# rhysnewell/Lorikeet

Measured on AMD Instinct MI355X. Metric: PairHMM cell-updates/s (GCUPS), higher is better.
Workload: dtype f64; 1 GPU; config2 x 1024 regions per GPU: 128 reads x 8 haps, R=150, H=300; regions_per_gpu=1024, seed=1000, env=PHMM_REGION_OWN_QUEUE=0 in this process only

## Files before the change

### lorikeet_amd/csrc/phmm_chain_kernels.hip

```cpp
#include "phmm_device.hpp"

namespace phmm {

namespace {

#ifndef PHMM_CHAIN_L
#define PHMM_CHAIN_L 16
#endif
constexpr int CL = PHMM_CHAIN_L;
#ifndef PHMM_RING
#define PHMM_RING 256
#endif
constexpr int RING = PHMM_RING;
constexpr int RING_SLOTS = RING + 4 + 1;
constexpr int CHAIN_META = CHAIN_MAX_READS + 8;
constexpr uint32_t X_PAD = 0x100u;
constexpr uint32_t X_NONE = 0x102u;
constexpr int LEAD = CL - 1;

__device__ __forceinline__ double from_left_inject(double v, double inject, bool group_head) {
    constexpr int ctrl = CL == 16 ? 0x111 : 0x138;
    int lo = __builtin_amdgcn_update_dpp(__double2loint(inject), __double2loint(v), ctrl, 0xf, 0xf, false);
    int hi = __builtin_amdgcn_update_dpp(__double2hiint(inject), __double2hiint(v), ctrl, 0xf, 0xf, false);
    if constexpr (CL == 32) {
        lo = group_head ? __double2loint(inject) : lo;
        hi = group_head ? __double2hiint(inject) : hi;
    }
    return __hiloint2double(hi, lo);
}

template <int K>
__device__ __forceinline__ void chain_fallback(const ForwardParams &p, const ChainItem &it, RowConst *ring, int lane,
                                               int grp, int l, const HapCols<K> &hc, int H, bool hv, int a, int Nh) {
    const uint32_t reg = it.region;
    for (uint32_t r = it.read_begin; r < it.read_end; ++r) {
        const uint32_t ro = p.read_off[r];
        const int R = (int)(p.read_off[r + 1] - ro);
        bool z = false;
        for (int row = lane; row < R; row += WAVE) z |= row_blocks_prescale(p, ro + row);
        const bool scaled = __ballot(z) == 0ull;
        const bool staged = R + 1 <= RING;
        lds_wave_sync();
        if (staged) {
            if (lane == 0) ring[0] = neutral_row();
            for (int row = lane; row < R; row += WAVE) ring[row + 1] = make_row(p, ro, row, R, scaled);
        }
        lds_wave_sync();
        const double scale0 = (scaled && R > 0) ? 1.0 - p.eps[p.gcp[ro]] : 1.0;
        const double fin = (scaled && R > 0) ? 1.0 - p.eps[p.base_q[ro + R - 1]] : 1.0;
        const double c0 = p.initial_condition / (double)H * scale0;
        const bool group_head = (CL == 32) && (lane == 32);
        double s = staged ? sweep_general<CL, K>(LdsView{ring}, R, l, group_head, hc, H, c0, scaled, fin)
                          : sweep_general<CL, K>(GlobalRowView{p, ro, R, scaled}, R, l, group_head, hc, H, c0, scaled, fin);
#pragma unroll
        for (int off = CL / 2; off > 0; off >>= 1) s += __shfl_xor(s, off, WAVE);
        if (l == 0 && hv) {
            const double v = log10(s) - p.initial_condition_log10;
            p.out[p.out_off[reg] + (uint64_t)(r - p.region_read_off[reg]) * (uint64_t)Nh + a] = v;
            if (const uint32_t sb = status_bits(v)) atomicOr(p.status, sb);
        }
    }
    (void)grp;
}

template <int K>
__device__ __forceinline__ void chain_fallback_streams(const ForwardParams &p, uint32_t reg, uint32_t r_begin, int n_mine,
                                                       int n_iter, int lane, int l, const HapCols<K> &hc, int H, bool hv,
                                                       int a, int Nh) {
    const uint64_t group_bits = 0xffffull << (lane & ~15);
    for (int i = 0; i < n_iter; ++i) {
        const bool valid = i < n_mine;
        const uint32_t r = r_begin + (uint32_t)i;
        const uint32_t ro = valid ? p.read_off[r] : 0u;
        const int R = valid ? (int)(p.read_off[r + 1] - ro) : 0;
        bool z = false;
        for (int row = l; row < R; row += 16) z |= row_blocks_prescale(p, ro + row);
        const bool scaled = (__ballot(z) & group_bits) == 0ull;
        const double scale0 = (scaled && R > 0) ? 1.0 - p.eps[p.gcp[ro]] : 1.0;
        const double fin = (scaled && R > 0) ? 1.0 - p.eps[p.base_q[ro + R - 1]] : 1.0;
        const double c0 = p.initial_condition / (double)H * scale0;
        double s = sweep_general<16, K>(GlobalRowView{p, ro, R, scaled}, R, l, false, hc, H, c0, scaled, fin);
#pragma unroll
        for (int off = 8; off > 0; off >>= 1) s += __shfl_xor(s, off, WAVE);
        if (l == 0 && hv && valid) {
            const double v = log10(s) - p.initial_condition_log10;
            p.out[p.out_off[reg] + (uint64_t)(r - p.region_read_off[reg]) * (uint64_t)Nh + a] = v;
            if (const uint32_t sb = status_bits(v)) atomicOr(p.status, sb);
        }
    }
}

}

template <int CLT, int K, int MODE = CHAIN_PLAIN>
__device__ __forceinline__ void chain_body(const ForwardParams &p, const ChainItem it, unsigned char *smem, const ChainItemX *x = nullptr,
                                           double *park = nullptr) {
    static_assert(CLT == CL, "one lanes-per-pair value per compilation unit");
    static_assert(MODE == CHAIN_PLAIN || CL == 16, "prefix sharing: 16 lanes per pair");
    const int col0 = MODE == CHAIN_SUFFIX ? (int)x->mask_or_col0 : 0;
    const uint32_t park_rows = MODE == CHAIN_PLAIN ? 0u : 16u * x->park_rows16;
    const uint32_t park_mask = MODE == CHAIN_PARK ? (uint32_t)x->mask_or_col0 : 0u;
    const int lane = threadIdx.x;
    const int grp = lane / CL, l = lane % CL;
    const bool group_head = (CL == 32) && (lane == 32);
    const uint32_t reg = it.region;
    const int n_chain = (int)(it.read_end - it.read_begin);
    const uint32_t h0 = p.region_hap_off[reg];
    const int Nh = (int)(p.region_hap_off[reg + 1] - h0);
    const int S = (CL == 16) ? (int)it.streams : 1;
    const int GS = (WAVE / CL) / S;
    const int sid = grp / GS;
    const int a = MODE == CHAIN_PLAIN ? (int)it.quad * GS + grp % GS : (int)x->hap[grp & 3];
    const bool hv = a < Nh;
    const int n_sub = (n_chain + S - 1) / S;
    const int TPS = (RING / 4) / S;
    const int NM = RING / S - 1;
    auto n_of = [&](int s) { return max(0, min(n_sub, n_chain - s * n_sub)); };
    const int n_mine = n_of(sid);
    uint32_t ho = 0;
    int H = 0;
    if (hv) {
        ho = p.hap_off[h0 + a];
        H = (int)(p.hap_off[h0 + a + 1] - ho);
    }
    RowConst *ring = reinterpret_cast<RowConst *>(smem);
    uint32_t *roff = reinterpret_cast<uint32_t *>(ring + RING_SLOTS);
    uint32_t *stot = roff + CHAIN_META;

    HapCols<K> hc;
    bool lane_n = false;
#pragma unroll
    for (int w = 0; w < HapCols<K>::W; ++w) hc.y[w] = 0u;
#pragma unroll
    for (int k = 0; k < K; ++k) {
        const int col = col0 + l * K + k;
        uint32_t y = col < H ? (uint32_t)p.hap_bases[ho + col] : X_PAD;
        const bool is_n = (y == 'N');
        lane_n |= is_n;
        hc.set(k, y);
    }

    const uint32_t rb = it.read_begin;
    const uint32_t byte0 = p.read_off[rb];
    const uint32_t bytes = p.read_off[it.read_end] - byte0;
    bool z = false;
    for (uint32_t i = lane; i < bytes; i += WAVE) z |= row_blocks_prescale(p, byte0 + i);
    if ((__ballot(z) | __ballot(lane_n)) != 0ull) {
        if constexpr (MODE == CHAIN_SUFFIX) {
            for (uint32_t r = rb + (uint32_t)l; r < it.read_end && hv; r += CL)
                p.out[p.out_off[reg] + (uint64_t)(r - p.region_read_off[reg]) * (uint64_t)Nh + a] = __longlong_as_double(0x7ff8000000000000ll);
            if (lane == 0) atomicOr(p.status, STATUS_RESCUE);
            return;
        }
        if (S == 1)
            chain_fallback<K>(p, it, ring, lane, grp, l, hc, H, hv, a, Nh);
        else if constexpr (CL == 16)
            chain_fallback_streams<K>(p, reg, rb + (uint32_t)(sid * n_sub), n_mine, n_sub, lane, l, hc, H, hv, a, Nh);
        return;
    }
    {
        const int sj = lane / n_sub, ij = lane % n_sub;
        uint32_t len = lane < n_chain ? p.read_off[rb + lane + 1] - p.read_off[rb + lane] + 2u : 0u;
        uint32_t incl = len;
#pragma unroll
        for (int off = 1; off < WAVE; off <<= 1) {
            const uint32_t v = __shfl_up(incl, off, WAVE);
            if (lane >= off) incl += v;
        }
        const uint32_t before = __shfl(incl, max(sj * n_sub - 1, 0), WAVE);
        const int cb = sj * (n_sub + 1);
        if (lane < 4) stot[lane] = 0u;
        if (lane < n_chain) {
            roff[cb + ij] = p.read_off[rb + lane];
            if (ij + 1 == n_of(sj)) {
                roff[cb + ij + 1] = p.read_off[rb + lane + 1];
                stot[sj] = incl - (sj > 0 ? before : 0u);
            }
        }
        if (lane == 0) ring[RING_SLOTS - 1] = neutral_row();
    }
    lds_wave_sync();
    const int S_max = (int)max(max(stot[0], stot[1]), max(stot[2], stot[3]));
    const double c_unit = ldexp(1.0, 1010);

    uint32_t pb_x = 0, pb_q = 0, pb_qp = 0, pb_i = 0, pb_d = 0, pb_dp = 0, pb_g = 0, pb_gn = 0;
    double pb_bM = 0.0, pb_bD = 0.0;
    int p_Q = 0;
    const bool producer = lane < S * TPS;
    const int ps = producer ? lane / TPS : 0, pj = lane % TPS;
    const int pcb = ps * (n_sub + 1), pn = n_of(ps);
    int p_lo = 0, p_row = pj - LEAD - TPS;
    p_Q = pj - TPS;
    uint32_t p_ro = pn > 0 ? roff[pcb] : 0u;
    int p_R = pn > 0 ? (int)(roff[pcb + 1] - p_ro) : 0;
    auto advance = [&]() {
        p_row += TPS;
        p_Q += TPS;
        while (p_lo < pn && p_row >= p_R + 2) {
            p_row -= p_R + 2;
            ++p_lo;
            if (p_lo < pn) {
                p_ro = roff[pcb + p_lo];
                p_R = (int)(roff[pcb + p_lo + 1] - p_ro);
            }
        }
    };
    auto issue = [&]() {
        advance();
        const int row = p_row, R = p_R;
        const uint32_t ro = p_ro;
        if constexpr (MODE == CHAIN_SUFFIX) {
            if (producer && p_lo < pn && row >= 0 && (uint32_t)p_Q < park_rows) {
                const double *at = park + 2 * ((size_t)x->park_row0 + (size_t)p_Q);
                pb_bM = at[0];
                pb_bD = at[1];
            }
        }
        if (producer && p_lo < pn && row >= 0 && row <= R) {
            pb_qp = row > 0 ? (uint32_t)p.base_q[ro + row - 1] : 0u;
            if (row < R) {
                pb_x = p.read_bases[ro + row];
                pb_q = p.base_q[ro + row];
                pb_i = p.ins_q[ro + row];
                pb_d = p.del_q[ro + row];
                pb_dp = row > 0 ? (uint32_t)p.del_q[ro + row - 1] : 0u;
                pb_g = p.gcp[ro + row];
                pb_gn = row + 1 < R ? (uint32_t)p.gcp[ro + row + 1] : 0u;
            }
        }
    };
    auto finish = [&](int Q0) {
        const int Q = Q0 + pj;
        const int lo = p_lo, row = p_row, R = p_R;
        RowConst n;
        if (lo < pn && row >= 0) {
            if (row < R) {
                n = make_row_bytes(p, pb_x, pb_q, pb_qp, pb_i, pb_d, pb_dp, pb_g, pb_gn, row == 0, row + 1 >= R, true);
            } else if (row == R) {
                n.mm = 1.0 - p.eps[pb_qp]; n.bI = n.mm; n.gI = 1.0; n.dDp = 0.0; n.dd = 1.0; n.pm = 1.0; n.px = 1.0;
                n.x = X_PAD; n.pad0 = (uint32_t)lo; n.pad1 = 0.0;
            } else {
                n.mm = 0.0; n.bI = 0.0; n.gI = 0.0; n.dDp = 0.0; n.dd = 1.0; n.pm = 0.0; n.px = 0.0;
                n.x = X_NONE; n.pad0 = 0;
                n.pad1 = c_unit * (lo + 1 < pn ? 1.0 - p.eps[p.gcp[roff[pcb + lo + 1]]] : 1.0);
            }
            if constexpr (MODE == CHAIN_SUFFIX) {
                n.pm = pb_bM;
                n.pad1 = pb_bD;
            }
        } else {
            n = neutral_row();
        }
        if (producer) {
            const int slot = ps * (NM + 2) + (Q & NM);
            ring[slot] = n;
            if ((Q & NM) == 0) ring[slot + NM + 1] = n;
        }
    };
    issue();
    finish(0);
    issue();
    finish(TPS);
    issue();
    finish(2 * TPS);
    lds_wave_sync();
    issue();

    const double c0 = c_unit * (n_mine > 0 ? 1.0 - p.eps[p.gcp[roff[sid * (n_sub + 1)]]] : 1.0);
    double Mp[K], Ip[K], Dp[K];
#pragma unroll
    for (int k = 0; k < K; ++k) {
        Mp[k] = 0.0;
        Ip[k] = 0.0;
        Dp[k] = c0;
    }
    double aM, aI, aD, bM = 0.0, bI = 0.0, bD = c0;
    const int edge_lane = (H > col0 ? H - 1 - col0 : 0) / K, edge_k = (H > col0 ? H - 1 - col0 : 0) % K;
    const bool last_lane = (l == edge_lane);
    const uint32_t sum_code = last_lane ? X_PAD : 0xffffffffu;
    const double log10_scale = log10(c_unit) + log10((double)H);
    auto emit = [&](const RowConst &c) {
        {
            if (last_lane && c.x == X_PAD && hv) {
                const uint32_t r = rb + (uint32_t)(sid * n_sub) + c.pad0;
                int ek = edge_k;
                asm volatile("" : "+v"(ek));
                double sum = 0.0;
#pragma unroll
                for (int k = 0; k < K; ++k)
                    if (k == ek) sum = (Dp[k] + Mp[k]) + Ip[k];
                const double v = log10(sum) - log10_scale;
                p.out[p.out_off[reg] + (uint64_t)(r - p.region_read_off[reg]) * (uint64_t)Nh + a] = v;
                if (const uint32_t sb = status_bits(v)) atomicOr(p.status, sb);
            }
        }
    };

    int q = LEAD - l;
    const int my_ring = sid * (NM + 2);
    const uint32_t my_rows = (uint32_t)(uintptr_t)(ring + my_ring);
    RowConst cA = lds_row(ring, my_ring + (q & NM)), cB;
    int q1 = q + 1;
    const int T = (S_max + CL - 1 + 1) & ~1;
    bool park_lane = false;
    double2 *park_at = nullptr;
    if constexpr (MODE == CHAIN_PARK) {
        park_lane = grp == 0 && ((park_mask >> l) & 1u) != 0u && hv && (uint32_t)(q + T) <= park_rows;
        const int b = __popc(park_mask & ((1u << l) - 1u));
        park_at = reinterpret_cast<double2 *>(park) + ((size_t)x->park_row0 + (size_t)b * park_rows + (size_t)q);
    }
    const int phase = (int)((blockIdx.x * 2654435761u) >> 26) & (TPS - 2);
    for (int t0 = 0, t1 = min(T, TPS - phase), tick = 0; t0 < T; t0 = t1, t1 = min(T, t1 + TPS), ++tick) {
        if (tick >= 1) {
            finish(TPS * tick + 2 * TPS);
            lds_wave_sync();
            issue();
        }
        for (int t = t0; t < t1; t += 2) {
            uint32_t pair_at;
            asm("v_mad_u32_u24 %0, %1, %2, %3" : "=v"(pair_at) : "v"((uint32_t)(q1 & NM)), "s"((uint32_t)sizeof(RowConst)), "v"(my_rows));
            cB = lds_row_at(pair_at, 0);
            if constexpr (MODE == CHAIN_SUFFIX) {
                aI = from_left_inject(Ip[K - 1], fma(bM, cA.bI, bI * cA.gI), group_head);
                aM = from_left_inject(Mp[K - 1], cA.pm, group_head);
            } else {
                aM = from_left<CL>(Mp[K - 1], group_head);
                aI = from_left<CL>(Ip[K - 1], group_head);
            }
            aD = from_left_inject(Dp[K - 1], cA.pad1, group_head);
            row_update<K, ROW_FAST_EXEC>(Mp, Ip, Dp, bM, bI, bD, aM, aD, cA, hc, 1.0);
            if constexpr (MODE == CHAIN_PARK)
                if (park_lane) park_at[0] = make_double2(Mp[K - 1], Dp[K - 1]);
            if (__ballot(cA.x == sum_code) != 0ull) emit(cA);
            cA = lds_row_at(pair_at, 1);
            if constexpr (MODE == CHAIN_SUFFIX) {
                bI = from_left_inject(Ip[K - 1], fma(aM, cB.bI, aI * cB.gI), group_head);
                bM = from_left_inject(Mp[K - 1], cB.pm, group_head);
            } else {
                bM = from_left<CL>(Mp[K - 1], group_head);
                bI = from_left<CL>(Ip[K - 1], group_head);
            }
            bD = from_left_inject(Dp[K - 1], cB.pad1, group_head);
            row_update<K, ROW_FAST_EXEC>(Mp, Ip, Dp, aM, aI, aD, bM, bD, cB, hc, 1.0);
            if constexpr (MODE == CHAIN_PARK) {
                if (park_lane) park_at[1] = make_double2(Mp[K - 1], Dp[K - 1]);
                park_at += 2;
            }
            if (__ballot(cB.x == sum_code) != 0ull) emit(cB);
            q1 += 2;
        }
    }
}


#define PHMM_CHAIN_K_LIST(X) \
    X(2) X(3) X(4) X(5) X(6) X(7) X(8) X(9) X(10) X(11) X(12) X(13) X(14) X(15) X(16) X(17) X(18) X(19) X(20) X(21) X(22) \
    X(23) X(24) X(25)

template <int CLT, int KLO, int KHI>
__global__ __launch_bounds__(WAVE, 2) void phmm_forward_chain(const ChainParams cp) {
    extern __shared__ __attribute__((aligned(16))) unsigned char smem[];
    const ChainItem it = cp.items[blockIdx.x];
    switch (__builtin_amdgcn_readfirstlane((int)it.k)) {
#define PHMM_CASE(KK)                                                  \
    case KK:                                                           \
        if constexpr (KK >= KLO && KK <= KHI) chain_body<CLT, KK>(cp.f, it, smem); \
        break;
        PHMM_CHAIN_K_LIST(PHMM_CASE)
#undef PHMM_CASE
        default:
            break;
    }
}

template <int CLT, int K>
__global__ __launch_bounds__(WAVE, 2) void phmm_forward_chain_k(const ChainParams cp) {
    extern __shared__ __attribute__((aligned(16))) unsigned char smem[];
    chain_body<CLT, K>(cp.f, cp.items[blockIdx.x], smem);
}

#define PHMM_CHAIN_CAT2(a, b) a##b
#define PHMM_CHAIN_CAT(a, b) PHMM_CHAIN_CAT2(a, b)
#define PHMM_CHAIN_LAUNCH PHMM_CHAIN_CAT(launch_chain_L, PHMM_CHAIN_L)

hipError_t PHMM_CHAIN_LAUNCH(int single_k, const ChainParams &cp, hipStream_t stream) {
    const size_t lds = (size_t)RING_SLOTS * sizeof(RowConst) + (CHAIN_META + 4) * sizeof(uint32_t);
#define PHMM_CASE(KK)                                                                                     \
    if (single_k == KK) {                                                                                 \
        hipLaunchKernelGGL((phmm_forward_chain_k<CL, KK>), dim3(cp.n_items), dim3(WAVE), lds, stream, cp); \
        return hipGetLastError();                                                                         \
    }
    PHMM_CHAIN_K_LIST(PHMM_CASE)
#undef PHMM_CASE
#define PHMM_RANGE(R, LO, HI)                                                                                       \
    if (single_k == -(R + 1)) {                                                                                     \
        hipLaunchKernelGGL((phmm_forward_chain<CL, LO, HI>), dim3(cp.n_items), dim3(WAVE), lds, stream, cp);        \
        return hipGetLastError();                                                                                   \
    }
    PHMM_CHAIN_RANGES(PHMM_RANGE)
#undef PHMM_RANGE
    return hipErrorInvalidValue;
}

#if PHMM_CHAIN_L == 16
hipError_t launch_chain_L32(int single_k, const ChainParams &cp, hipStream_t stream);
hipError_t launch_chain_L64(int single_k, const ChainParams &cp, hipStream_t stream);
int chain_max_k() { return 25; }
hipError_t launch_chain(int L, int single_k, const ChainParams &cp, hipStream_t stream) {
    if (!cp.n_items) return hipSuccess;
    return L == 16 ? launch_chain_L16(single_k, cp, stream) : L == 32 ? launch_chain_L32(single_k, cp, stream)
         : L == 64 ? launch_chain_L64(single_k, cp, stream) : hipErrorInvalidValue;
}
#endif

}
```

### lorikeet_amd/csrc/phmm_device.hpp

```cpp
#pragma once
#include "phmm_internal.hpp"

#include <type_traits>

#ifndef PHMM_SDWA_MIN_K
#define PHMM_SDWA_MIN_K 21
#endif
#ifndef PHMM_CND_MAX_K
#define PHMM_CND_MAX_K 13
#endif
#ifndef PHMM_TWO_WAVE_MAX_K
#define PHMM_TWO_WAVE_MAX_K 25
#endif

namespace phmm {

__device__ __forceinline__ int dpp_row_shr1(int v) {
    return __builtin_amdgcn_update_dpp(0, v, 0x111, 0xf, 0xf, true);
}
__device__ __forceinline__ int dpp_wave_shr1(int v) {
    return __builtin_amdgcn_update_dpp(0, v, 0x138, 0xf, 0xf, true);
}

template <int L>
__device__ __forceinline__ double from_left(double v, bool group_head) {
    int lo = __double2loint(v), hi = __double2hiint(v);
    if constexpr (L == 16) {
        lo = dpp_row_shr1(lo);
        hi = dpp_row_shr1(hi);
    } else {
        lo = dpp_wave_shr1(lo);
        hi = dpp_wave_shr1(hi);
        if constexpr (L == 32) {
            lo = group_head ? 0 : lo;
            hi = group_head ? 0 : hi;
        }
    }
    return __hiloint2double(hi, lo);
}

struct alignas(8) RowConst {
    double mm, bI, gI, dDp, dd, pm, px;
    uint32_t x, pad0;
    double pad1;
};
static_assert(sizeof(RowConst) == 72, "LDS row record");

__device__ __forceinline__ RowConst lds_row(const RowConst *rows, int idx) {
    return *reinterpret_cast<const RowConst *>(reinterpret_cast<const unsigned char *>(rows) +
                                               __mul24(idx, (int)sizeof(RowConst)));
}

__device__ __forceinline__ RowConst lds_row_at(uint32_t at, int skip) {
    RowConst r;
#if defined(__HIP_DEVICE_COMPILE__)
    typedef const __attribute__((address_space(3))) unsigned long long *LdsU64;
    const LdsU64 w = (LdsU64)(uintptr_t)at + skip * (int)(sizeof(RowConst) / 8);
    unsigned long long v[sizeof(RowConst) / 8];
#pragma unroll
    for (int i = 0; i < (int)(sizeof(RowConst) / 8) - 1; ++i) v[i] = w[i];
    v[8] = w[8];
    __builtin_memcpy(&r, v, sizeof r);
#else
    (void)at;
    (void)skip;
    r = RowConst{};
#endif
    return r;
}

struct LdsView {
    const RowConst *rows;
    __device__ __forceinline__ RowConst load(int idx) const { return lds_row(rows, idx); }
};

template <int K, class F>
__device__ __forceinline__ void static_for_down(F &&f) {
    if constexpr (K > 0) {
        f(std::integral_constant<int, K - 1>{});
        static_for_down<K - 1>(f);
    }
}

template <int K>
struct HapCols {
    static constexpr int W = (K + 1) / 2;
    uint32_t y[W];
    __device__ __forceinline__ uint16_t base(int k) const { return (uint16_t)(y[k >> 1] >> (16 * (k & 1))); }
    __device__ __forceinline__ void set(int k, uint32_t yv) { y[k >> 1] |= yv << (16 * (k & 1)); }
};

enum : int { ROW_GENERAL = 0, ROW_FAST_CND = 1, ROW_FAST_EXEC = 2, ROW_FAST_EXEC_PRED = 3 };

template <int K, int MODE>
__device__ __forceinline__ void row_update(double (&Mp)[K], double (&Ip)[K], double (&Dp)[K], const double plM,
                                           const double plI, const double plD, const double lM, const double lD,
                                           const RowConst &c, const HapCols<K> &hc, const double imx,
                                           const uint64_t live = ~0ull) {
    const uint16_t x16 = (uint16_t)c.x;
    if constexpr (MODE == ROW_FAST_EXEC || MODE == ROW_FAST_EXEC_PRED) {
        const uint64_t restore = (MODE == ROW_FAST_EXEC) ? ~0ull : live;
        constexpr bool packed = K > PHMM_SDWA_MIN_K;
        constexpr bool pred = MODE == ROW_FAST_EXEC_PRED;
        uint64_t mask;
        {
            constexpr int k = K - 1;
            const uint32_t y = packed ? hc.y[k >> 1] : (uint32_t)hc.base(k);
            if constexpr (packed && (k & 1))
                asm volatile("v_cmp_ne_u32_sdwa %0, %1, %2 src0_sel:DWORD src1_sel:WORD_1" : "=s"(mask) : "v"(c.x), "v"(y));
            else if constexpr (packed)
                asm volatile("v_cmp_ne_u32_sdwa %0, %1, %2 src0_sel:DWORD src1_sel:WORD_0" : "=s"(mask) : "v"(c.x), "v"(y));
            else
                asm volatile("v_cmp_ne_u32_e64 %0, %1, %2" : "=s"(mask) : "v"(c.x), "v"(y));
        }
        Ip[K - 1] = fma(Mp[K - 1], c.bI, Ip[K - 1] * c.gI);
        static_for_down<K>([&](auto kc) {
            constexpr int k = decltype(kc)::value;
            constexpr int km1 = k > 0 ? k - 1 : 0;
            const uint32_t yn = packed ? hc.y[km1 >> 1] : (uint32_t)hc.base(km1);
            uint64_t next;
#define PHMM_CELL(CMP, RESTORE)                                                                                      \
    asm volatile("v_fma_f64 %[M], %[Dl], %[dDp], %[Il]\n\t"                                                        \
                 "v_fma_f64 %[M], %[Ml], %[mm], %[M]\n\t"                                                          \
                 "s_mov_b64 exec, %[mk]\n\t"                                                                       \
                 "v_mul_f64 %[M], %[px], %[M]\n\t"                                                                 \
                 "s_mov_b64 exec, " RESTORE "\n\t"                                                                 \
                 CMP "\n\t"                                                                                      \
                 "v_mul_f64 %[Il], %[Il], %[gI]\n\t"                                                               \
                 "v_fma_f64 %[Il], %[Ml], %[bI], %[Il]"                                                             \
                 : [M] "=&v"(Mp[k]), [Il] "+v"(Ip[km1]), [mn] "=&s"(next)                                           \
                 : [Dl] "v"(Dp[km1]), [dDp] "v"(c.dDp), [Ml] "v"(Mp[km1]), [mm] "v"(c.mm), [x] "v"(c.x), [y] "v"(yn), \
                   [px] "v"(c.px), [gI] "v"(c.gI), [bI] "v"(c.bI), [live] "s"(restore), [mk] "s"(mask))
            if constexpr (k > 0 && pred && packed && (km1 & 1)) {
                PHMM_CELL("v_cmp_ne_u32_sdwa %[mn], %[x], %[y] src0_sel:DWORD src1_sel:WORD_1", "%[live]");
            } else if constexpr (k > 0 && pred && packed) {
                PHMM_CELL("v_cmp_ne_u32_sdwa %[mn], %[x], %[y] src0_sel:DWORD src1_sel:WORD_0", "%[live]");
            } else if constexpr (k > 0 && pred) {
                PHMM_CELL("v_cmp_ne_u32_e64 %[mn], %[x], %[y]", "%[live]");
            } else if constexpr (k > 0 && packed && (km1 & 1)) {
                PHMM_CELL("v_cmp_ne_u32_sdwa %[mn], %[x], %[y] src0_sel:DWORD src1_sel:WORD_1", "-1");
            } else if constexpr (k > 0 && packed) {
                PHMM_CELL("v_cmp_ne_u32_sdwa %[mn], %[x], %[y] src0_sel:DWORD src1_sel:WORD_0", "-1");
            } else if constexpr (k > 0) {
                PHMM_CELL("v_cmp_ne_u32_e64 %[mn], %[x], %[y]", "-1");
#undef PHMM_CELL
            } else {
                (void)yn;
                double m = fma(plM, c.mm, fma(plD, c.dDp, plI));
                asm volatile("s_mov_b64 exec, %2\n\t"
                             "v_mul_f64 %0, %1, %0\n\t"
                             "s_mov_b64 exec, %3"
                             : "+v"(m)
                             : "v"(c.px), "s"(mask), "s"(restore));
                Mp[0] = m;
                next = 0;
            }
            mask = next;
        });
        double leftM = lM, leftD = lD;
#pragma unroll
        for (int k = 0; k < K; ++k) {
            Dp[k] = fma(leftD, c.dd, leftM);
            leftM = Mp[k];
            leftD = Dp[k];
        }
        return;
    }
    static_for_down<K>([&](auto kc) {
        constexpr int k = decltype(kc)::value;
        Ip[k] = fma(Mp[k], c.bI, Ip[k] * c.gI);
        constexpr int km1 = k > 0 ? k - 1 : 0;
        const double dM = k > 0 ? Mp[km1] : plM;
        const double dI = k > 0 ? Ip[km1] : plI;
        const double dD = k > 0 ? Dp[km1] : plD;
        double t = fma(dD, c.dDp, dI);
        if constexpr (MODE == ROW_GENERAL) t *= imx;
        const double a = fma(dM, c.mm, t);
        const uint16_t yb = hc.base(k);
        const double prior = (x16 == yb || (MODE == ROW_GENERAL && yb == (uint16_t)'N')) ? c.pm : c.px;
        Mp[k] = prior * a;
    });
    double leftM = lM, leftD = lD;
#pragma unroll
    for (int k = 0; k < K; ++k) {
        Dp[k] = fma(leftD, c.dd, leftM);
        leftM = Mp[k];
        leftD = Dp[k];
    }
}


template <int L, int K, int STEADY = ROW_FAST_EXEC>
__device__ __forceinline__ double sweep_fast(const LdsView &lds, const int R, const int l, const bool group_head,
                                             const HapCols<K> &hc, const int H, const double c0, const double fin) {
    double Mp[K], Ip[K], Dp[K];
#pragma unroll
    for (int k = 0; k < K; ++k) {
        Mp[k] = 0.0;
        Ip[k] = 0.0;
        Dp[k] = c0;
    }
    double aM, aI, aD, bM = 0.0, bI = 0.0, bD = c0;
    int row = -l;
    RowConst cA = lds.load(max(row + 1, 0)), cB;
    int t = 0;
    for (; t + 1 < R; t += 2) {
        cB = lds.load(max(row + 2, 0));
        aM = from_left<L>(Mp[K - 1], group_head);
        aI = from_left<L>(Ip[K - 1], group_head);
        aD = from_left<L>(Dp[K - 1], group_head);
        row_update<K, STEADY>(Mp, Ip, Dp, bM, bI, bD, aM, aD, cA, hc, 1.0);
        cA = lds.load(max(row + 3, 0));
        bM = from_left<L>(Mp[K - 1], group_head);
        bI = from_left<L>(Ip[K - 1], group_head);
        bD = from_left<L>(Dp[K - 1], group_head);
        row_update<K, STEADY>(Mp, Ip, Dp, aM, aI, aD, bM, bD, cB, hc, 1.0);
        row += 2;
    }
    RowConst cur = cA;
    double plM = bM, plI = bI, plD = bD;
    if (t < R) {
        const RowConst nxt = lds.load(max(row + 2, 0));
        const double lM = from_left<L>(Mp[K - 1], group_head);
        const double lI = from_left<L>(Ip[K - 1], group_head);
        const double lD = from_left<L>(Dp[K - 1], group_head);
        row_update<K, STEADY>(Mp, Ip, Dp, plM, plI, plD, lM, lD, cur, hc, 1.0);
        plM = lM;
        plI = lI;
        plD = lD;
        ++row;
        cur = nxt;
    }
    for (int d = 0; d < L - 1; ++d) {
        const RowConst nxt = lds.load(max(min(row + 2, R), 0));
        const double lM = from_left<L>(Mp[K - 1], group_head);
        const double lI = from_left<L>(Ip[K - 1], group_head);
        const double lD = from_left<L>(Dp[K - 1], group_head);
        const uint64_t live = __ballot(row < R);
        if (row < R)
            row_update<K, STEADY == ROW_FAST_CND ? ROW_FAST_CND : ROW_FAST_EXEC_PRED>(Mp, Ip, Dp, plM, plI, plD, lM, lD, cur,
                                                                                     hc, 1.0, live);
        plM = lM;
        plI = lI;
        plD = lD;
        ++row;
        cur = nxt;
    }
    double s = 0.0;
#pragma unroll
    for (int k = 0; k < K; ++k)
        if (l * K + k < H) s += fma(Mp[k], fin, Ip[k]);
    return s;
}

template <int L, int K, class RowView>
__device__ __forceinline__ double sweep_general(const RowView &lds, const int R, const int l, const bool group_head,
                                             const HapCols<K> &hc, const int H, const double c0, const bool scaled,
                                             const double fin) {
    double Mp[K], Ip[K], Dp[K];
#pragma unroll
    for (int k = 0; k < K; ++k) {
        Mp[k] = 0.0;
        Ip[k] = 0.0;
        Dp[k] = c0;
    }
    double plM = 0.0, plI = 0.0, plD = c0;
    int row = -l;
    for (int t = 0; t < R + L - 1; ++t) {
        const RowConst cur = lds.load(max(min(row + 1, R), 0));
        const double lM = from_left<L>(Mp[K - 1], group_head);
        const double lI = from_left<L>(Ip[K - 1], group_head);
        const double lD = from_left<L>(Dp[K - 1], group_head);
        const double imx = scaled ? 1.0 : 1.0 - cur.dd;
        if (row < R) row_update<K, ROW_GENERAL>(Mp, Ip, Dp, plM, plI, plD, lM, lD, cur, hc, imx);
        plM = lM;
        plI = lI;
        plD = lD;
        ++row;
    }
    double s = 0.0;
#pragma unroll
    for (int k = 0; k < K; ++k)
        if (l * K + k < H) s += fma(Mp[k], fin, Ip[k]);
    return s;
}


__device__ __forceinline__ RowConst make_row_bytes(const ForwardParams &p, uint32_t x, uint32_t q, uint32_t q_prev,
                                                   uint32_t iq, uint32_t dq, uint32_t dq_prev, uint32_t g,
                                                   uint32_t g_next, bool first, bool last, bool scaled) {
    const double mi = p.eps[iq], ii = p.eps[g];
    const uint32_t mx = max(iq, dq), mn = min(iq, dq);
    const double mm = p.mm[((mx * (mx + 1)) >> 1) + mn];
    RowConst n;
    n.dd = ii;
    if (scaled) {
        const double im = 1.0 - ii;
        const double im_next = last ? 1.0 : 1.0 - p.eps[g_next];
        const double pm_prev = first ? 1.0 : 1.0 - p.eps[q_prev];
        n.mm = mm * pm_prev;
        n.bI = mi * im_next * pm_prev;
        n.gI = ii * (im_next * p.inv_om[g]);
        n.dDp = first ? 1.0 : p.eps[dq_prev] * im * pm_prev;
        n.pm = 1.0;
        n.px = (x == 'N') ? 1.0 : p.ratio_mis[q];
    } else {
        const double pm = 1.0 - p.eps[q];
        const double px = (x == 'N') ? pm : p.eps_mis[q];
        n.mm = mm;
        n.bI = mi;
        n.gI = ii;
        n.dDp = first ? 1.0 : p.eps[dq_prev];
        n.pm = pm;
        n.px = px;
    }
    n.x = x;
    n.pad0 = 0;
    n.pad1 = 0.0;
    return n;
}

__device__ __forceinline__ RowConst make_row(const ForwardParams &p, uint32_t ro, int row, int R, bool scaled) {
    const bool first = row == 0, last = row + 1 >= R;
    return make_row_bytes(p, p.read_bases[ro + row], p.base_q[ro + row], first ? 0u : (uint32_t)p.base_q[ro + row - 1],
                          p.ins_q[ro + row], p.del_q[ro + row], first ? 0u : (uint32_t)p.del_q[ro + row - 1],
                          p.gcp[ro + row], last ? 0u : (uint32_t)p.gcp[ro + row + 1], first, last, scaled);
}

__device__ __forceinline__ RowConst neutral_row();

struct GlobalRowView {
    const ForwardParams &p;
    uint32_t ro;
    int R;
    bool scaled;
    __device__ __forceinline__ RowConst load(int idx) const {
        return idx == 0 ? neutral_row() : make_row(p, ro, idx - 1, R, scaled);
    }
};

__device__ __forceinline__ bool row_blocks_prescale(const ForwardParams &p, uint32_t byte) {
    return p.gcp[byte] == 0 || p.base_q[byte] == 0;
}

__device__ __forceinline__ RowConst neutral_row() {
    RowConst n;
    n.mm = 0.0; n.bI = 0.0; n.gI = 1.0; n.dDp = 0.0; n.dd = 1.0; n.pm = 0.0; n.px = 0.0;
    n.x = 0; n.pad0 = 0; n.pad1 = 0.0;
    return n;
}

__device__ __forceinline__ void lds_wave_sync() {
    __builtin_amdgcn_fence(__ATOMIC_RELEASE, "wavefront");
    __builtin_amdgcn_wave_barrier();
    __builtin_amdgcn_fence(__ATOMIC_ACQUIRE, "wavefront");
}

template <int L, int K>
__device__ __forceinline__ void forward_read(const ForwardParams &p, const uint32_t r, const int quad_begin, const int quad_step,
                                             const bool cnd_select, unsigned char *smem_wave, double *coherent_out = nullptr) {
    constexpr int G = WAVE / L;
    const int lane = threadIdx.x & (WAVE - 1);
    const int grp = lane / L, l = lane % L;
    const uint32_t reg = p.read_region[r];
    const uint32_t ro = p.read_off[r];
    const int R = (int)(p.read_off[r + 1] - ro);
    const uint32_t h0 = p.region_hap_off[reg];
    const int Nh = (int)(p.region_hap_off[reg + 1] - h0);
    double *out_row = p.out + p.out_off[reg] + (uint64_t)(r - p.region_read_off[reg]) * (uint64_t)Nh;

    RowConst *srow = reinterpret_cast<RowConst *>(smem_wave);
    bool lane_zero_gcp = false;
    for (int row = lane; row < R; row += WAVE) lane_zero_gcp |= row_blocks_prescale(p, ro + row);
    const bool scaled = __ballot(lane_zero_gcp) == 0ull;
    if (lane == 0) srow[0] = neutral_row();
    for (int row = lane; row < R; row += WAVE) srow[row + 1] = make_row(p, ro, row, R, scaled);
    const double scale0 = (scaled && R > 0) ? 1.0 - p.eps[p.gcp[ro]] : 1.0;
    const double fin = (scaled && R > 0) ? 1.0 - p.eps[p.base_q[ro + R - 1]] : 1.0;
    lds_wave_sync();
    const LdsView lds{srow};
    const bool group_head = (L == 32) && (lane == 32);

    const int nquads = (Nh + G - 1) / G;
    for (int quad = quad_begin; quad < nquads; quad += quad_step) {
        const int a = quad * G + grp;
        const bool hv = a < Nh;
        uint32_t ho = 0;
        int H = 0;
        if (hv) {
            ho = p.hap_off[h0 + a];
            H = (int)(p.hap_off[h0 + a + 1] - ho);
        }
        HapCols<K> hc;
        bool lane_n = false;
#pragma unroll
        for (int w = 0; w < HapCols<K>::W; ++w) hc.y[w] = 0u;
#pragma unroll
        for (int k = 0; k < K; ++k) {
            const int col = l * K + k;
            const uint32_t y = (col < H) ? (uint32_t)p.hap_bases[ho + col] : 0u;
            const bool is_n = (y == 'N');
            lane_n |= is_n;
            hc.set(k, y);
        }
        const double c0 = p.initial_condition / (double)H * scale0;
        double s;
        if (scaled && __ballot(lane_n) == 0ull) {
            if constexpr (K <= PHMM_CND_MAX_K) {
                s = cnd_select ? sweep_fast<L, K, ROW_FAST_CND>(lds, R, l, group_head, hc, H, c0, fin)
                               : sweep_fast<L, K>(lds, R, l, group_head, hc, H, c0, fin);
            } else {
                s = sweep_fast<L, K>(lds, R, l, group_head, hc, H, c0, fin);
            }
        } else {
            s = sweep_general<L, K>(lds, R, l, group_head, hc, H, c0, scaled, fin);
        }
#pragma unroll
        for (int off = L / 2; off > 0; off >>= 1) s += __shfl_xor(s, off, WAVE);
        if (l == 0 && hv) {
            const double v = log10(s) - p.initial_condition_log10;
            if (coherent_out) __hip_atomic_store(&coherent_out[a], v, __ATOMIC_RELAXED, __HIP_MEMORY_SCOPE_AGENT);
            else out_row[a] = v;
            if (const uint32_t sb = status_bits(v)) atomicOr(p.status, sb);
        }
    }
}

}
```

### lorikeet_amd/csrc/phmm_internal.hpp

```cpp
#pragma once
#include <hip/hip_runtime.h>
#include <stdint.h>

namespace phmm {

constexpr int WAVE = 64;
constexpr int MAX_WAVES_PER_BLOCK = 4;
constexpr int KMAX = 32;
constexpr int LDS_ROW_BYTES = 72;

struct ForwardParams {
    const uint32_t *class_reads;
    uint32_t n_items;
    const uint32_t *read_region;
    const uint32_t *region_read_off;
    const uint32_t *region_hap_off;
    const uint32_t *read_off;
    const uint32_t *hap_off;
    const uint64_t *out_off;
    const uint8_t *read_bases, *base_q, *ins_q, *del_q, *gcp, *hap_bases;
    double *out;
    const double *eps;
    const double *eps_mis;
    const double *mm;
    const double *ratio_mis;
    const double *inv_om;
    double initial_condition;
    double initial_condition_log10;
    uint32_t lds_rows;
    const uint8_t *redo;
    uint32_t pad_was_priority;
    uint32_t cnd_select;
    uint32_t *status;
};

constexpr uint32_t STATUS_POSITIVE = 1u;
constexpr uint32_t STATUS_RESCUE = 2u;
constexpr uint32_t STATUS_POSITIVE_FINAL = 4u;
__host__ __device__ inline bool status_positive(uint32_t bits, bool rescue_rides_inline) {
    return rescue_rides_inline && (bits & STATUS_RESCUE) ? (bits & STATUS_POSITIVE_FINAL) != 0 : (bits & STATUS_POSITIVE) != 0;
}
constexpr double kRescueBelow = -600.0;
__host__ __device__ inline uint32_t status_bits(double v) {
    return (!(v <= 0.0) ? STATUS_POSITIVE : 0u) | (!(v >= kRescueBelow) ? STATUS_RESCUE : 0u);
}

hipError_t launch_forward(int L, int K, const ForwardParams &p, dim3 grid, int waves_per_block, size_t lds_bytes,
                          hipStream_t stream);
struct GenericParams {
    ForwardParams f;
    double *scratch;
    uint32_t max_h;
    const uint64_t *pair_first;
    uint64_t n_pairs;
    uint32_t n_blocks;
};
hipError_t launch_generic(const GenericParams &p, hipStream_t stream);

struct RescueParams {
    ForwardParams f;
    uint32_t n_reads;
    double *scratch;
    uint32_t max_h;
    uint32_t n_blocks;
    uint32_t force;
};
hipError_t launch_rescue(const RescueParams &p, hipStream_t stream);
inline void rescue_geometry(uint32_t max_h, uint32_t *n_blocks, size_t *scratch_bytes) {
    const size_t per_thread = 6ull * ((size_t)max_h + 1) * sizeof(double);
    size_t threads = (64ull << 20) / per_thread / 64 * 64;
    threads = threads < 64 ? 64 : threads > 4096 ? 4096 : threads;
    *n_blocks = (uint32_t)(threads / 64);
    *scratch_bytes = threads * per_thread;
}

constexpr int CHAIN_MAX_READS = 64;
struct ChainItem {
    uint32_t region;
    uint16_t quad;
    uint8_t k, streams;
    uint32_t read_begin, read_end;
};
static_assert(sizeof(ChainItem) == 16, "work item record");
struct ChainParams {
    ForwardParams f;
    const ChainItem *items;
    uint32_t n_items;
    uint8_t *redo;
};
enum : int { CHAIN_PLAIN = 0, CHAIN_PARK = 1, CHAIN_SUFFIX = 2 };
struct ChainItemX {
    ChainItem it;
    uint16_t hap[4];
    uint32_t park_row0;
    uint16_t park_rows16;
    uint16_t mask_or_col0;
};
static_assert(sizeof(ChainItemX) == 32, "work item record");
#define PHMM_CHAIN_RANGES(X) X(0, 2, 9) X(1, 10, 15) X(2, 16, 19) X(3, 20, 25)
constexpr int kChainRanges = 4;
constexpr int chain_range_of(int k) { return k <= 9 ? 0 : k <= 15 ? 1 : k <= 19 ? 2 : 3; }
hipError_t launch_chain(int L, int single_k, const ChainParams &p, hipStream_t stream);
hipError_t launch_chain_f32(int L, int single_k, const ChainParams &p, hipStream_t stream);
int chain_max_k();

struct PrepParams {
    uint32_t n_reads;
    const uint32_t *read_off;
    const uint8_t *read_bases, *base_q, *ins_q, *del_q;
    const uint8_t *mapq;
    const uint8_t *pcr_cache;
    uint8_t *out_q, *out_ins, *out_del, *out_gcp;
    double *threshold;
    uint32_t lds_rows;
    uint32_t waves_per_read;
    uint32_t default_indel_qual, constant_gcp, base_quality_score_threshold, disable_cap_to_mapq,
        dynamic_disqualification;
    double read_disqualification_scale, expected_error_rate_per_base;
    const void *stage_src;
    void *stage_dst;
    uint32_t stage_n16;
};
struct PostParams {
    uint32_t n_reads;
    const uint32_t *read_region, *region_read_off, *region_hap_off;
    const uint64_t *out_off;
    const int32_t *region_ref_hap;
    double *out;
    double *out_final;
    const double *threshold;
    uint8_t *keep;
    const uint32_t *status_in;
    uint32_t *status_out;
    double max_likelihood_difference_cap;
    uint32_t symmetric;
};
hipError_t launch_prep(const PrepParams &p, hipStream_t stream);
hipError_t launch_post(const PostParams &p, hipStream_t stream);
constexpr uint32_t SW_NO_REFERENCE = 0xffffffffu;
struct BestParams {
    uint32_t r_begin, n_reads, n_regions;
    const uint32_t *region_read_off, *region_hap_off;
    const uint64_t *out_off;
    const double *likelihoods;
    const uint8_t *keep;
    const int32_t *priority;
    double threshold;
    int32_t *best_allele;
    double *likelihood, *confidence;
    uint32_t *ref_index;
};
hipError_t launch_best_alleles(const BestParams &p, hipStream_t stream);
struct PostBestParams {
    PostParams post;
    BestParams best;
    uint32_t skip_single_allele;
    uint8_t *keep_final;
};
hipError_t launch_post_best(const PostBestParams &p, hipStream_t stream);

extern const int kInstantiatedK[];
extern const int kNumInstantiatedK;

}
```

Before: 4551 GCUPS.

## Split D-chain from row update, predict emit ticks, and drop prefix-sharing modes

Removes the PARK/SUFFIX prefix-sharing modes from the chain kernel. The inner loop is restructured: the row update no longer runs the serial D chain inline. Instead the pad1 inject value is loaded separately as a scalar LDS read, and the D chain runs after the DPP inject, which is meant to shorten the dependency chain and overlap LDS latency. The per-row ballot that decided when to emit results is replaced by precomputed due ticks per lane with a scalar compare. Small inline-asm rewrites of the I and M cell updates are also included.

Result: no change. 4572 GCUPS, median of 6 (+0.4%).

```diff
diff --git a/lorikeet_amd/csrc/phmm_chain_kernels.hip b/lorikeet_amd/csrc/phmm_chain_kernels.hip
--- a/lorikeet_amd/csrc/phmm_chain_kernels.hip
+++ b/lorikeet_amd/csrc/phmm_chain_kernels.hip
@@ -92,14 +92,9 @@
 
 }
 
-template <int CLT, int K, int MODE = CHAIN_PLAIN>
-__device__ __forceinline__ void chain_body(const ForwardParams &p, const ChainItem it, unsigned char *smem, const ChainItemX *x = nullptr,
-                                           double *park = nullptr) {
+template <int CLT, int K>
+__device__ __forceinline__ void chain_body(const ForwardParams &p, const ChainItem it, unsigned char *smem) {
     static_assert(CLT == CL, "one lanes-per-pair value per compilation unit");
-    static_assert(MODE == CHAIN_PLAIN || CL == 16, "prefix sharing: 16 lanes per pair");
-    const int col0 = MODE == CHAIN_SUFFIX ? (int)x->mask_or_col0 : 0;
-    const uint32_t park_rows = MODE == CHAIN_PLAIN ? 0u : 16u * x->park_rows16;
-    const uint32_t park_mask = MODE == CHAIN_PARK ? (uint32_t)x->mask_or_col0 : 0u;
     const int lane = threadIdx.x;
     const int grp = lane / CL, l = lane % CL;
     const bool group_head = (CL == 32) && (lane == 32);
@@ -110,7 +105,7 @@
     const int S = (CL == 16) ? (int)it.streams : 1;
     const int GS = (WAVE / CL) / S;
     const int sid = grp / GS;
-    const int a = MODE == CHAIN_PLAIN ? (int)it.quad * GS + grp % GS : (int)x->hap[grp & 3];
+    const int a = (int)it.quad * GS + grp % GS;
     const bool hv = a < Nh;
     const int n_sub = (n_chain + S - 1) / S;
     const int TPS = (RING / 4) / S;
@@ -133,7 +128,7 @@
     for (int w = 0; w < HapCols<K>::W; ++w) hc.y[w] = 0u;
 #pragma unroll
     for (int k = 0; k < K; ++k) {
-        const int col = col0 + l * K + k;
+        const int col = l * K + k;
         uint32_t y = col < H ? (uint32_t)p.hap_bases[ho + col] : X_PAD;
         const bool is_n = (y == 'N');
         lane_n |= is_n;
@@ -146,12 +141,6 @@
     bool z = false;
     for (uint32_t i = lane; i < bytes; i += WAVE) z |= row_blocks_prescale(p, byte0 + i);
     if ((__ballot(z) | __ballot(lane_n)) != 0ull) {
-        if constexpr (MODE == CHAIN_SUFFIX) {
-            for (uint32_t r = rb + (uint32_t)l; r < it.read_end && hv; r += CL)
-                p.out[p.out_off[reg] + (uint64_t)(r - p.region_read_off[reg]) * (uint64_t)Nh + a] = __longlong_as_double(0x7ff8000000000000ll);
-            if (lane == 0) atomicOr(p.status, STATUS_RESCUE);
-            return;
-        }
         if (S == 1)
             chain_fallback<K>(p, it, ring, lane, grp, l, hc, H, hv, a, Nh);
         else if constexpr (CL == 16)
@@ -184,7 +173,6 @@
     const double c_unit = ldexp(1.0, 1010);
 
     uint32_t pb_x = 0, pb_q = 0, pb_qp = 0, pb_i = 0, pb_d = 0, pb_dp = 0, pb_g = 0, pb_gn = 0;
-    double pb_bM = 0.0, pb_bD = 0.0;
     int p_Q = 0;
     const bool producer = lane < S * TPS;
     const int ps = producer ? lane / TPS : 0, pj = lane % TPS;
@@ -209,13 +197,6 @@
         advance();
         const int row = p_row, R = p_R;
         const uint32_t ro = p_ro;
-        if constexpr (MODE == CHAIN_SUFFIX) {
-            if (producer && p_lo < pn && row >= 0 && (uint32_t)p_Q < park_rows) {
-                const double *at = park + 2 * ((size_t)x->park_row0 + (size_t)p_Q);
-                pb_bM = at[0];
-                pb_bD = at[1];
-            }
-        }
         if (producer && p_lo < pn && row >= 0 && row <= R) {
             pb_qp = row > 0 ? (uint32_t)p.base_q[ro + row - 1] : 0u;
             if (row < R) {
@@ -238,15 +219,11 @@
                 n = make_row_bytes(p, pb_x, pb_q, pb_qp, pb_i, pb_d, pb_dp, pb_g, pb_gn, row == 0, row + 1 >= R, true);
             } else if (row == R) {
                 n.mm = 1.0 - p.eps[pb_qp]; n.bI = n.mm; n.gI = 1.0; n.dDp = 0.0; n.dd = 1.0; n.pm = 1.0; n.px = 1.0;
-                n.x = X_PAD; n.pad0 = (uint32_t)lo; n.pad1 = 0.0;
+                n.x = X_PAD; n.pad0 = 0; n.pad1 = 0.0;
             } else {
                 n.mm = 0.0; n.bI = 0.0; n.gI = 0.0; n.dDp = 0.0; n.dd = 1.0; n.pm = 0.0; n.px = 0.0;
                 n.x = X_NONE; n.pad0 = 0;
                 n.pad1 = c_unit * (lo + 1 < pn ? 1.0 - p.eps[p.gcp[roff[pcb + lo + 1]]] : 1.0);
-            }
-            if constexpr (MODE == CHAIN_SUFFIX) {
-                n.pm = pb_bM;
-                n.pad1 = pb_bD;
             }
         } else {
             n = neutral_row();
@@ -266,7 +243,8 @@
     lds_wave_sync();
     issue();
 
-    const double c0 = c_unit * (n_mine > 0 ? 1.0 - p.eps[p.gcp[roff[sid * (n_sub + 1)]]] : 1.0);
+    const int cb = sid * (n_sub + 1);
+    const double c0 = c_unit * (n_mine > 0 ? 1.0 - p.eps[p.gcp[roff[cb]]] : 1.0);
     double Mp[K], Ip[K], Dp[K];
 #pragma unroll
     for (int k = 0; k < K; ++k) {
@@ -275,40 +253,62 @@
         Dp[k] = c0;
     }
     double aM, aI, aD, bM = 0.0, bI = 0.0, bD = c0;
-    const int edge_lane = (H > col0 ? H - 1 - col0 : 0) / K, edge_k = (H > col0 ? H - 1 - col0 : 0) % K;
-    const bool last_lane = (l == edge_lane);
-    const uint32_t sum_code = last_lane ? X_PAD : 0xffffffffu;
+    const int edge_lane = (H > 0 ? H - 1 : 0) / K, edge_k = (H > 0 ? H - 1 : 0) % K;
     const double log10_scale = log10(c_unit) + log10((double)H);
-    auto emit = [&](const RowConst &c) {
-        {
-            if (last_lane && c.x == X_PAD && hv) {
-                const uint32_t r = rb + (uint32_t)(sid * n_sub) + c.pad0;
+    constexpr int NO_DUE = 0x7fffffff;
+    int emit_lane[WAVE / CL];
+#pragma unroll
+    for (int g = 0; g < WAVE / CL; ++g) emit_lane[g] = g * CL + __builtin_amdgcn_readlane(edge_lane, g * CL);
+    int e_read = 0;
+    int due = (l == edge_lane && hv && n_mine > 0) ? (int)(roff[cb + 1] - roff[cb]) + l : NO_DUE;
+    auto earliest = [&]() {
+        int m = NO_DUE;
+#pragma unroll
+        for (int g = 0; g < WAVE / CL; ++g) m = min(m, __builtin_amdgcn_readlane(due, emit_lane[g]));
+        return __builtin_amdgcn_readfirstlane(m);
+    };
+    int next_due = earliest();
+    const uint64_t hv_lanes = __ballot(hv);
+    const int edge_k0 = __builtin_amdgcn_readlane(edge_k, hv_lanes ? (int)__builtin_ctzll(hv_lanes) : 0);
+    const bool edge_k_uniform = __ballot(hv && edge_k != edge_k0) == 0ull;
+    auto emit = [&](const int t) {
+        if (due == t) {
+            const uint32_t r = rb + (uint32_t)(sid * n_sub + e_read);
+            double sum = 0.0;
+            if (edge_k_uniform) {
+                int ek = edge_k0;
+                asm volatile("" : "+s"(ek));
+#pragma unroll
+                for (int k = 0; k < K; ++k)
+                    if (ek == k)
+                        asm volatile("v_add_f64 %0, %1, %2\n\t"
+                                     "v_add_f64 %0, %0, %3"
+                                     : "=&v"(sum)
+                                     : "v"(Dp[k]), "v"(Mp[k]), "v"(Ip[k]));
+            } else {
                 int ek = edge_k;
                 asm volatile("" : "+v"(ek));
-                double sum = 0.0;
 #pragma unroll
                 for (int k = 0; k < K; ++k)
                     if (k == ek) sum = (Dp[k] + Mp[k]) + Ip[k];
-                const double v = log10(sum) - log10_scale;
-                p.out[p.out_off[reg] + (uint64_t)(r - p.region_read_off[reg]) * (uint64_t)Nh + a] = v;
-                if (const uint32_t sb = status_bits(v)) atomicOr(p.status, sb);
             }
-        }
+            const double v = log10(sum) - log10_scale;
+            p.out[p.out_off[reg] + (uint64_t)(r - p.region_read_off[reg]) * (uint64_t)Nh + a] = v;
+            if (const uint32_t sb = status_bits(v)) atomicOr(p.status, sb);
+            ++e_read;
+            due = e_read < n_mine ? due + (int)(roff[cb + e_read + 1] - roff[cb + e_read]) + 2 : NO_DUE;
+        }
+        next_due = earliest();
     };
 
     int q = LEAD - l;
     const int my_ring = sid * (NM + 2);
     const uint32_t my_rows = (uint32_t)(uintptr_t)(ring + my_ring);
     RowConst cA = lds_row(ring, my_ring + (q & NM)), cB;
+    constexpr int PAD1 = (int)offsetof(RowConst, pad1);
+    double injA = cA.pad1, injB;
     int q1 = q + 1;
     const int T = (S_max + CL - 1 + 1) & ~1;
-    bool park_lane = false;
-    double2 *park_at = nullptr;
-    if constexpr (MODE == CHAIN_PARK) {
-        park_lane = grp == 0 && ((park_mask >> l) & 1u) != 0u && hv && (uint32_t)(q + T) <= park_rows;
-        const int b = __popc(park_mask & ((1u << l) - 1u));
-        park_at = reinterpret_cast<double2 *>(park) + ((size_t)x->park_row0 + (size_t)b * park_rows + (size_t)q);
-    }
     const int phase = (int)((blockIdx.x * 2654435761u) >> 26) & (TPS - 2);
     for (int t0 = 0, t1 = min(T, TPS - phase), tick = 0; t0 < T; t0 = t1, t1 = min(T, t1 + TPS), ++tick) {
         if (tick >= 1) {
@@ -319,34 +319,24 @@
         for (int t = t0; t < t1; t += 2) {
             uint32_t pair_at;
             asm("v_mad_u32_u24 %0, %1, %2, %3" : "=v"(pair_at) : "v"((uint32_t)(q1 & NM)), "s"((uint32_t)sizeof(RowConst)), "v"(my_rows));
-            cB = lds_row_at(pair_at, 0);
-            if constexpr (MODE == CHAIN_SUFFIX) {
-                aI = from_left_inject(Ip[K - 1], fma(bM, cA.bI, bI * cA.gI), group_head);
-                aM = from_left_inject(Mp[K - 1], cA.pm, group_head);
-            } else {
-                aM = from_left<CL>(Mp[K - 1], group_head);
-                aI = from_left<CL>(Ip[K - 1], group_head);
-            }
-            aD = from_left_inject(Dp[K - 1], cA.pad1, group_head);
-            row_update<K, ROW_FAST_EXEC>(Mp, Ip, Dp, bM, bI, bD, aM, aD, cA, hc, 1.0);
-            if constexpr (MODE == CHAIN_PARK)
-                if (park_lane) park_at[0] = make_double2(Mp[K - 1], Dp[K - 1]);
-            if (__ballot(cA.x == sum_code) != 0ull) emit(cA);
-            cA = lds_row_at(pair_at, 1);
-            if constexpr (MODE == CHAIN_SUFFIX) {
-                bI = from_left_inject(Ip[K - 1], fma(aM, cB.bI, aI * cB.gI), group_head);
-                bM = from_left_inject(Mp[K - 1], cB.pm, group_head);
-            } else {
-                bM = from_left<CL>(Mp[K - 1], group_head);
-                bI = from_left<CL>(Ip[K - 1], group_head);
-            }
-            bD = from_left_inject(Dp[K - 1], cB.pad1, group_head);
-            row_update<K, ROW_FAST_EXEC>(Mp, Ip, Dp, aM, aI, aD, bM, bD, cB, hc, 1.0);
-            if constexpr (MODE == CHAIN_PARK) {
-                if (park_lane) park_at[1] = make_double2(Mp[K - 1], Dp[K - 1]);
-                park_at += 2;
-            }
-            if (__ballot(cB.x == sum_code) != 0ull) emit(cB);
+            cB = lds_row_at<false>(pair_at, 0);
+            aM = from_left<CL>(Mp[K - 1], group_head);
+            aI = from_left<CL>(Ip[K - 1], group_head);
+            row_update<K, ROW_FAST_EXEC, false>(Mp, Ip, Dp, bM, bI, bD, 0.0, 0.0, cA, hc, 1.0);
+            asm volatile("" ::: "memory");
+            injB = lds_f64_at(pair_at, PAD1);
+            aD = from_left_inject(Dp[K - 1], injA, group_head);
+            row_dchain<K>(Mp, Dp, aM, aD, cA.dd);
+            if (t == next_due) emit(t);
+            cA = lds_row_at<false>(pair_at, 1);
+            bM = from_left<CL>(Mp[K - 1], group_head);
+            bI = from_left<CL>(Ip[K - 1], group_head);
+            row_update<K, ROW_FAST_EXEC, false>(Mp, Ip, Dp, aM, aI, aD, 0.0, 0.0, cB, hc, 1.0);
+            asm volatile("" ::: "memory");
+            injA = lds_f64_at(pair_at, (int)sizeof(RowConst) + PAD1);
+            bD = from_left_inject(Dp[K - 1], injB, group_head);
+            row_dchain<K>(Mp, Dp, bM, bD, cB.dd);
+            if (t + 1 == next_due) emit(t + 1);
             q1 += 2;
         }
     }
diff --git a/lorikeet_amd/csrc/phmm_device.hpp b/lorikeet_amd/csrc/phmm_device.hpp
--- a/lorikeet_amd/csrc/phmm_device.hpp
+++ b/lorikeet_amd/csrc/phmm_device.hpp
@@ -51,6 +51,7 @@
                                                __mul24(idx, (int)sizeof(RowConst)));
 }
 
+template <bool PAD1 = true>
 __device__ __forceinline__ RowConst lds_row_at(uint32_t at, int skip) {
     RowConst r;
 #if defined(__HIP_DEVICE_COMPILE__)
@@ -59,7 +60,7 @@
     unsigned long long v[sizeof(RowConst) / 8];
 #pragma unroll
     for (int i = 0; i < (int)(sizeof(RowConst) / 8) - 1; ++i) v[i] = w[i];
-    v[8] = w[8];
+    v[8] = PAD1 ? w[8] : 0ull;
     __builtin_memcpy(&r, v, sizeof r);
 #else
     (void)at;
@@ -69,6 +70,16 @@
     return r;
 }
 
+__device__ __forceinline__ double lds_f64_at(uint32_t at, int off) {
+#if defined(__HIP_DEVICE_COMPILE__)
+    return *(const __attribute__((address_space(3))) double *)(uintptr_t)(at + (uint32_t)off);
+#else
+    (void)at;
+    (void)off;
+    return 0.0;
+#endif
+}
+
 struct LdsView {
     const RowConst *rows;
     __device__ __forceinline__ RowConst load(int idx) const { return lds_row(rows, idx); }
@@ -92,7 +103,19 @@
 
 enum : int { ROW_GENERAL = 0, ROW_FAST_CND = 1, ROW_FAST_EXEC = 2, ROW_FAST_EXEC_PRED = 3 };
 
-template <int K, int MODE>
+template <int K>
+__device__ __forceinline__ void row_dchain(const double (&Mp)[K], double (&Dp)[K], const double lM, const double lD,
+                                           const double dd) {
+    double leftM = lM, leftD = lD;
+#pragma unroll
+    for (int k = 0; k < K; ++k) {
+        Dp[k] = fma(leftD, dd, leftM);
+        leftM = Mp[k];
+        leftD = Dp[k];
+    }
+}
+
+template <int K, int MODE, bool DCHAIN = true>
 __device__ __forceinline__ void row_update(double (&Mp)[K], double (&Ip)[K], double (&Dp)[K], const double plM,
                                            const double plI, const double plD, const double lM, const double lD,
                                            const RowConst &c, const HapCols<K> &hc, const double imx,
@@ -113,7 +136,10 @@
             else
                 asm volatile("v_cmp_ne_u32_e64 %0, %1, %2" : "=s"(mask) : "v"(c.x), "v"(y));
         }
-        Ip[K - 1] = fma(Mp[K - 1], c.bI, Ip[K - 1] * c.gI);
+        asm volatile("v_mul_f64 %0, %0, %2\n\t"
+                     "v_fma_f64 %0, %1, %3, %0"
+                     : "+v"(Ip[K - 1])
+                     : "v"(Mp[K - 1]), "v"(c.gI), "v"(c.bI));
         static_for_down<K>([&](auto kc) {
             constexpr int k = decltype(kc)::value;
             constexpr int km1 = k > 0 ? k - 1 : 0;
@@ -146,26 +172,22 @@
 #undef PHMM_CELL
             } else {
                 (void)yn;
-                double m = fma(plM, c.mm, fma(plD, c.dDp, plI));
-                asm volatile("s_mov_b64 exec, %2\n\t"
-                             "v_mul_f64 %0, %1, %0\n\t"
-                             "s_mov_b64 exec, %3"
-                             : "+v"(m)
-                             : "v"(c.px), "s"(mask), "s"(restore));
-                Mp[0] = m;
+                asm volatile("v_fma_f64 %[M], %[Dl], %[dDp], %[Il]\n\t"
+                             "v_fma_f64 %[M], %[Ml], %[mm], %[M]\n\t"
+                             "s_mov_b64 exec, %[mk]\n\t"
+                             "v_mul_f64 %[M], %[px], %[M]\n\t"
+                             "s_mov_b64 exec, %[live]"
+                             : [M] "=&v"(Mp[0])
+                             : [Dl] "v"(plD), [dDp] "v"(c.dDp), [Il] "v"(plI), [Ml] "v"(plM), [mm] "v"(c.mm), [px] "v"(c.px),
+                               [mk] "s"(mask), [live] "s"(restore));
                 next = 0;
             }
             mask = next;
         });
-        double leftM = lM, leftD = lD;
-#pragma unroll
-        for (int k = 0; k < K; ++k) {
-            Dp[k] = fma(leftD, c.dd, leftM);
-            leftM = Mp[k];
-            leftD = Dp[k];
-        }
+        if constexpr (DCHAIN) row_dchain<K>(Mp, Dp, lM, lD, c.dd);
         return;
     }
+    static_assert(DCHAIN || MODE == ROW_FAST_EXEC || MODE == ROW_FAST_EXEC_PRED, "the other forms run the D chain");
     static_for_down<K>([&](auto kc) {
         constexpr int k = decltype(kc)::value;
         Ip[k] = fma(Mp[k], c.bI, Ip[k] * c.gI);
@@ -180,13 +202,7 @@
         const double prior = (x16 == yb || (MODE == ROW_GENERAL && yb == (uint16_t)'N')) ? c.pm : c.px;
         Mp[k] = prior * a;
     });
-    double leftM = lM, leftD = lD;
-#pragma unroll
-    for (int k = 0; k < K; ++k) {
-        Dp[k] = fma(leftD, c.dd, leftM);
-        leftM = Mp[k];
-        leftD = Dp[k];
-    }
+    row_dchain<K>(Mp, Dp, lM, lD, c.dd);
 }
 
 
diff --git a/lorikeet_amd/csrc/phmm_internal.hpp b/lorikeet_amd/csrc/phmm_internal.hpp
--- a/lorikeet_amd/csrc/phmm_internal.hpp
+++ b/lorikeet_amd/csrc/phmm_internal.hpp
@@ -88,15 +88,6 @@
     uint32_t n_items;
     uint8_t *redo;
 };
-enum : int { CHAIN_PLAIN = 0, CHAIN_PARK = 1, CHAIN_SUFFIX = 2 };
-struct ChainItemX {
-    ChainItem it;
-    uint16_t hap[4];
-    uint32_t park_row0;
-    uint16_t park_rows16;
-    uint16_t mask_or_col0;
-};
-static_assert(sizeof(ChainItemX) == 32, "work item record");
 #define PHMM_CHAIN_RANGES(X) X(0, 2, 9) X(1, 10, 15) X(2, 16, 19) X(3, 20, 25)
 constexpr int kChainRanges = 4;
 constexpr int chain_range_of(int k) { return k <= 9 ? 0 : k <= 15 ? 1 : k <= 19 ? 2 : 3; }
```
